# VealFang/PLI-SLAM

Measured on AMD Instinct MI355X. Metric: stereo frames/sec (ORB+LSD extract+match), 752x480 EuRoC, higher is better.
Workload: dtype u8; 1 GPU; 1xMI355X: 752x480 stereo pairs, extract + stereo Hamming match (BASELINE configs[1] shape, batched); 752x480, 1200 ORB kp (8 levels x1.2) + LSD/LBD (<=100 lines); 256 stereo frames per GPU per step; frames_per_gpu=256, parallelism=frame-batch data parallel, 1 rank(s), gather of result tables to rank 0

## Files before the change

### pli_slam_amd/csrc/kernels.hpp

```cpp
#pragma once
#include "common.hpp"

namespace pli {

struct BlurPlane {
  int w, h, pitchIn, pitchOut;
  int64_t offIn, offOut;
  int tilesX, tileBase;
};
struct BlurJob {
  int nplanes;
  BlurPlane pl[MAX_LEVELS];
  int k[7];
  int radius;
};
struct LbdCoef { float L[21]; float G[63]; };

constexpr signed char ORB_PATTERN_HOST[1024] = {
#include "../../include/pli_orb_pattern.inc"
};
constexpr int orbPatternReach() {
  int best = 0;
  for (int i = 0; i < 512; ++i) {
    const long long x = ORB_PATTERN_HOST[2 * i], y = ORB_PATTERN_HOST[2 * i + 1], r2 = x * x + y * y;
    int n = 0;
    while ((long long)(2 * n + 1) * (2 * n + 1) * 10000 <= 4 * r2 * 10002) ++n;
    best = n > best ? n : best;
  }
  return best;
}
constexpr int ORB_REACH = orbPatternReach();
constexpr int ORB_BLUR_R = 3;
constexpr int ORB_HALF_PATCH = 15;
constexpr int LBD_BLUR_R = 2;
constexpr int PROJ_K = 64;
__global__ void k_ingest_copy16(const uint8_t* __restrict__ left, const uint8_t* __restrict__ right, int64_t stride, int64_t frameStride, uint8_t* __restrict__ pyr, int64_t pyrBlock, int W16, int H, int pitch, int img0);
__global__ void k_ingest(const uint8_t* __restrict__ left, const uint8_t* __restrict__ right, int64_t stride, int64_t frameStride, uint8_t* __restrict__ pyr, int64_t pyrBlock, int W, int H, int pitch, const float2* __restrict__ mapL, const float2* __restrict__ mapR, int img0);
__global__ void k_resize_level(const uint8_t* __restrict__ srcBase, int64_t srcImgStride, int sw, int sh, int spitch, uint8_t* __restrict__ dstBase, int64_t dstImgStride, int dw, int dh, int dpitch, const int* __restrict__ tab, int img0);
__global__ void k_fast_cells(const DevParams* __restrict__ Pp, const uint8_t* __restrict__ pyr, uint32_t* __restrict__ cellCand, int* __restrict__ cellCount, int img0);
__global__ void k_octree(const DevParams* __restrict__ Pp, const uint32_t* __restrict__ cellCand, const int* __restrict__ cellCount, uint32_t* __restrict__ candAll, unsigned short* __restrict__ nodeOfAll, int* __restrict__ candCount, uint32_t* __restrict__ kpSel, int* __restrict__ kpSelCount, int img0);
__global__ void k_octree_512(const DevParams* __restrict__ Pp, const uint32_t* __restrict__ cellCand, const int* __restrict__ cellCount, uint32_t* __restrict__ candAll, unsigned short* __restrict__ nodeOfAll, int* __restrict__ candCount, uint32_t* __restrict__ kpSel, int* __restrict__ kpSelCount, int img0);
__global__ void k_octree_320(const DevParams* __restrict__ Pp, const uint32_t* __restrict__ cellCand, const int* __restrict__ cellCount, uint32_t* __restrict__ candAll, unsigned short* __restrict__ nodeOfAll, int* __restrict__ candCount, uint32_t* __restrict__ kpSel, int* __restrict__ kpSelCount, int img0);
__global__ void k_octree_w(const DevParams* __restrict__ Pp, const uint32_t* __restrict__ cellCand, const int* __restrict__ cellCount, uint32_t* __restrict__ candAll, unsigned short* __restrict__ nodeOfAll, int* __restrict__ candCount, uint32_t* __restrict__ kpSel, int* __restrict__ kpSelCount, int img0);
__global__ void k_octree_512_w(const DevParams* __restrict__ Pp, const uint32_t* __restrict__ cellCand, const int* __restrict__ cellCount, uint32_t* __restrict__ candAll, unsigned short* __restrict__ nodeOfAll, int* __restrict__ candCount, uint32_t* __restrict__ kpSel, int* __restrict__ kpSelCount, int img0);
__global__ void k_octree_320_w(const DevParams* __restrict__ Pp, const uint32_t* __restrict__ cellCand, const int* __restrict__ cellCount, uint32_t* __restrict__ candAll, unsigned short* __restrict__ nodeOfAll, int* __restrict__ candCount, uint32_t* __restrict__ kpSel, int* __restrict__ kpSelCount, int img0);
__global__ void k_blur(const BlurJob* __restrict__ Jp, const uint8_t* __restrict__ in, int64_t inImgStride, uint8_t* __restrict__ out, int64_t outImgStride, int img0);
__global__ void k_describe(const DevParams* __restrict__ Pp, const uint8_t* __restrict__ pyr, const BlurJob* __restrict__ Jp, const uint32_t* __restrict__ kpSel, const int* __restrict__ kpSelCount, uint8_t* __restrict__ table, int64_t recordBytes, int64_t offCounts, int64_t offKp0, int64_t offKp1, int64_t offDesc0, int64_t offDesc1, int img0);
__global__ void k_kp_counts(const DevParams* __restrict__ Pp, const int* __restrict__ kpSelCount, uint8_t* __restrict__ table, int64_t recordBytes, int64_t offCounts, int nimg, int img0);
__global__ void k_lsd_grad(const uint8_t* __restrict__ scaled, int64_t imgStride, int W, int H, int WP, int pitch, int g2Thresh, float4* __restrict__ rec, int* __restrict__ g2o, int2* __restrict__ own, int* __restrict__ maxG2, float* __restrict__ angDbg, int img0, int trigF32);
__global__ void k_lsd_hist(const int* __restrict__ g2a, int npix, int g2Thresh, int nBins, const int* __restrict__ maxG2, unsigned short* __restrict__ chunkHist, int nChunks, int img0, const double* __restrict__ mgAll, const unsigned long long* __restrict__ maxMg, double rho, const RxCtl* __restrict__ onlyUnsettled);
__global__ void k_lsd_scan(const unsigned short* __restrict__ chunkHist, int nChunks, int nBins, int* __restrict__ chunkBase, int* __restrict__ nDefined, int img0, const RxCtl* __restrict__ onlyUnsettled);
__global__ void k_lsd_scatter(const int* __restrict__ g2a, int npix, int g2Thresh, int nBins, const int* __restrict__ maxG2, const int* __restrict__ chunkBase, int nChunks, int* __restrict__ order, int img0, int nimg, const double* __restrict__ mgAll, const unsigned long long* __restrict__ maxMg, double rho, int* __restrict__ rankAll, const int* __restrict__ groupOff, int chunksPerGroup, int nGroups, const RxCtl* __restrict__ onlyUnsettled);
__global__ void k_lsd_scan_part(const unsigned short* __restrict__ chunkHist, int nChunks, int nBins, int chunksPerGroup, int* __restrict__ chunkBase, int* __restrict__ groupOff, int img0, const RxCtl* __restrict__ onlyUnsettled);
__global__ void k_lsd_scan_groups(int nGroups, int nBins, int* __restrict__ groupOff, int* __restrict__ nDefined, int img0, const RxCtl* __restrict__ onlyUnsettled);
__global__ void k_lsd_grow_unsettled(const DevParams* __restrict__ Pp, float4* __restrict__ recAll, const double* __restrict__ mgAll, const int* __restrict__ orderAll, const int* __restrict__ nDefined, uint2* __restrict__ regOverflow, float* __restrict__ segAll, int* __restrict__ nSeg, int maxSeg, int img0, int nimg, RxCtl* __restrict__ ctl);
__global__ void k_lsd_grow(const DevParams* __restrict__ Pp, float4* __restrict__ recAll, const double* __restrict__ mgAll, const int* __restrict__ orderAll, const int* __restrict__ nDefined, uint2* __restrict__ regOverflow, float* __restrict__ segAll, int* __restrict__ nSeg, int maxSeg, int img0, int nimg);
__global__ void k_lsd_grow2(const DevParams* __restrict__ Pp, float4* __restrict__ recAll, const double* __restrict__ mgAll, const int* __restrict__ orderAll, const int* __restrict__ nDefined, uint2* __restrict__ regOverflow, float* __restrict__ segAll, int* __restrict__ nSeg, int maxSeg, int img0, int nimg);
__global__ void k_lsd_grow_spec(const DevParams* __restrict__ Pp, float4* __restrict__ recAll, const double* __restrict__ mgAll, const int* __restrict__ orderAll, const int* __restrict__ nDefined, uint2* __restrict__ regOverflow, float* __restrict__ segAll, int* __restrict__ nSeg, int maxSeg, int img0, int nimg, LsdRectItem* __restrict__ rectAll, double* __restrict__ rectWAll);
__global__ void k_lsd_grow2_spec(const DevParams* __restrict__ Pp, float4* __restrict__ recAll, const double* __restrict__ mgAll, const int* __restrict__ orderAll, const int* __restrict__ nDefined, uint2* __restrict__ regOverflow, float* __restrict__ segAll, int* __restrict__ nSeg, int maxSeg, int img0, int nimg, LsdRectItem* __restrict__ rectAll, double* __restrict__ rectWAll);
__global__ void k_lsd_rect(const DevParams* __restrict__ Pp, const LsdRectItem* __restrict__ rectAll, const uint2* __restrict__ arenaAll, const double* __restrict__ mgAll, const double* __restrict__ rectWAll, const int* __restrict__ nSeg, float* __restrict__ segAll, int maxSeg, int img0);
__global__ void k_keylines(const DevParams* __restrict__ Pp, const float* __restrict__ seg, const int* __restrict__ nSeg, int maxSeg, pli_keyline* __restrict__ tmpKL, uint8_t* __restrict__ table, int64_t recordBytes, int64_t offCounts, int64_t offKl0, int64_t offKl1, int img0);
__global__ void k_sobel(const BlurJob* __restrict__ Jp, const uint8_t* __restrict__ in, int64_t inImgStride, short2* __restrict__ dxy, int img0);
__global__ void k_lbd(const DevParams* __restrict__ Pp, const LbdCoef* __restrict__ coef, const short2* __restrict__ dxya, uint8_t* __restrict__ table, int64_t recordBytes, int64_t offCounts, int64_t offKl0, int64_t offKl1, int64_t offLd0, int64_t offLd1, float* __restrict__ dbgFloat, int img0);
__global__ void k_lsd_blur64(const uint8_t* __restrict__ pyr, int64_t pyrBlock, int W, int H, int pitch, const double* __restrict__ kern, int radius, double* __restrict__ out, int64_t outImgStride, int img0);
__global__ void k_lsd_resize64(const double* __restrict__ src, int sw, int sh, double* __restrict__ dst, int dw, int dh, int64_t dstImgStride, const int* __restrict__ tab, int img0);
__global__ void k_lsd_grad64(const double* __restrict__ scaled, int W, int H, int WP, int64_t scaledImgStride, double rho, float4* __restrict__ rec, double* __restrict__ mg, int2* __restrict__ own, unsigned long long* __restrict__ maxMg, float* __restrict__ angDbg, int img0, int flags, int2* __restrict__ hot, float2* __restrict__ cold);
__global__ void k_lsd_front64(const uint8_t* __restrict__ pyr, int64_t pyrBlock, int sw, int sh, int pitch, const double* __restrict__ kern, int radius, const int* __restrict__ tab, int dw, int dh, int dp, double rho, float4* __restrict__ rec, double* __restrict__ mg, int2* __restrict__ own, unsigned long long* __restrict__ maxMg, int img0, int flags, int2* __restrict__ hot, float2* __restrict__ cold);
__global__ void k_rx_guess(const float4* __restrict__ recAll, const int* __restrict__ rankAll, int2* __restrict__ ownAll, int W, int H, float precDeg, int img0);
__global__ void k_rx_diff(RxCtl* __restrict__ ctl, const int2* __restrict__ ownAll, int* __restrict__ tileMinAll, int* __restrict__ tileActAll, int W, int H, int TW, int TH, int t, int img0, const int* __restrict__ tileTouchAll);
__global__ void k_rx_classify(RxCtl* __restrict__ ctl, const int2* __restrict__ ownAll, const int* __restrict__ rankAll, const int2* __restrict__ rgBoxAll, uint8_t* __restrict__ rgCleanAll, const int* __restrict__ tileMinAll, int W, int H, int TW, int TH, int t, int img0);
__global__ void k_rx_seed(RxCtl* __restrict__ ctl, int2* __restrict__ ownAll, const int* __restrict__ rankAll, const float4* __restrict__ recAll, const int* __restrict__ rgSizeAll, const uint8_t* __restrict__ rgCleanAll, RxSeed* __restrict__ smallAll, RxSeed* __restrict__ bigAll, int bigCap, int W, int H, int bigThresh, int t, int img0);
__global__ void k_rx_mark(RxCtl* __restrict__ ctl, const int2* __restrict__ ownAll, const int* __restrict__ rankAll, const int2* __restrict__ rgBoxAll, int* __restrict__ rgDirtyAll, const int* __restrict__ tileMinAll, int* __restrict__ tileActAll, int W, int H, int TW, int TH, int t, int img0, int seedRule, const int* __restrict__ rgLostAll, TxDirtyLists DL);
__global__ void k_rx_seed_sparse(RxCtl* __restrict__ ctl, int2* __restrict__ ownAll, const int* __restrict__ rankAll, const float4* __restrict__ recAll, const int* __restrict__ rgSizeAll, const int* __restrict__ rgDirtyAll, const int* __restrict__ tileActAll, RxSeed* __restrict__ smallAll, RxSeed* __restrict__ bigAll, int bigCap, int W, int H, int TW, int TH, int bigThresh, int t, int img0);
__global__ void k_rx_grow(const DevParams* __restrict__ Pp, RxCtl* __restrict__ ctl, const float4* __restrict__ recAll, int2* __restrict__ ownAll, const RxSeed* __restrict__ smallAll, int* __restrict__ rgSizeAll, int2* __restrict__ rgBoxAll, RxHand* __restrict__ handAll, int handCap, int* __restrict__ arenaAll, int arenaCap, RxRect* __restrict__ rectAll, int rectCap, int img0, int t);
__global__ void k_rx_grow_big(const DevParams* __restrict__ Pp, RxCtl* __restrict__ ctl, const float4* __restrict__ recAll, int2* __restrict__ ownAll, const RxSeed* __restrict__ bigAll, int bigCap, const RxHand* __restrict__ handAll, int handCap, int* __restrict__ rgSizeAll, int2* __restrict__ rgBoxAll, int* __restrict__ arenaAll, int arenaCap, RxRect* __restrict__ rectAll, int rectCap, int img0, int t);
__global__ void k_rx_grow_wave(const DevParams* __restrict__ Pp, RxCtl* __restrict__ ctl, const float4* __restrict__ recAll, int2* __restrict__ ownAll, const RxSeed* __restrict__ bigAll, int bigCap, const RxHand* __restrict__ handAll, int handCap, int* __restrict__ rgSizeAll, int2* __restrict__ rgBoxAll, int* __restrict__ arenaAll, int arenaCap, RxRect* __restrict__ rectAll, int rectCap, int img0, int t);
__global__ void k_rx_rect(const DevParams* __restrict__ Pp, RxCtl* __restrict__ ctl, const float4* __restrict__ recAll, const int* __restrict__ arenaAll, int arenaCap, const RxRect* __restrict__ rectAll, int rectCap, float4* __restrict__ rgSegAll, int img0, const double* __restrict__ mgAll, int rmask, const int2* __restrict__ hotAll, const float2* __restrict__ coldAll);
__global__ void k_rx_count(const RxCtl* __restrict__ ctl, const int* __restrict__ orderAll, const int* __restrict__ nDefined, const int2* __restrict__ ownAll, const int* __restrict__ rgSizeAll, int* __restrict__ chunkCntAll, int nChunks, int64_t npix, int minReg, int img0);
__global__ void k_rx_emit(const RxCtl* __restrict__ ctl, const int* __restrict__ orderAll, const int* __restrict__ nDefined, const int2* __restrict__ ownAll, const int* __restrict__ rgSizeAll, const float4* __restrict__ rgSegAll, const int* __restrict__ chunkCntAll, int nChunks, int64_t npix, int minReg, float* __restrict__ segAll, int* __restrict__ nSeg, int maxSeg, int img0);
__global__ void k_tx_sort(const int* __restrict__ rankAll, const int* __restrict__ orderAll, int2* __restrict__ ownAll, int2* __restrict__ listAll, int* __restrict__ tileCntAll, int W, int H, int ts, int ntx, int nty, int img0, TxKeys keys);
__global__ void k_tx_sort128(const int* __restrict__ rankAll, const int* __restrict__ orderAll, int2* __restrict__ ownAll, int2* __restrict__ listAll, int* __restrict__ tileCntAll, int W, int H, int ts, int ntx, int nty, int img0, TxKeys keys);
__global__ void k_tx_mark(RxCtl* __restrict__ ctl, const int2* __restrict__ ownAll, const int* __restrict__ rankAll, const int2* __restrict__ rgBoxAll, int* __restrict__ rgDirtyAll, const int* __restrict__ tileMinAll, int* __restrict__ tileActAll, int W, int H, int TW, int TH, int t, int img0, const int* __restrict__ rgLostAll, TxDirtyLists DL);
__global__ void k_tx_round2(RxCtl* __restrict__ ctl, int2* __restrict__ ownAll, const int* __restrict__ rankAll, const int* __restrict__ orderAll, const int2* __restrict__ rgBoxAll, int* __restrict__ rgDirtyAll, int* __restrict__ tileActAll, int W, int H, int TW, int TH, int t, int img0, const int* __restrict__ rgLostAll, TxDirtyLists DL, int* __restrict__ tileTouchAll, const float4* __restrict__ recPack, int keepRect, const int2* __restrict__ hotPack);
__global__ void k_tx_reset_rect(RxCtl* __restrict__ ctl, int nimg, int img0);
__global__ void k_tx_diffmark(RxCtl* __restrict__ ctl, const int2* __restrict__ ownAll, const int* __restrict__ rankAll, const int2* __restrict__ rgBoxAll, int* __restrict__ rgDirtyAll, int* __restrict__ tileActAll, const int* __restrict__ tileTouchAll, int W, int H, int TW, int TH, int t, int img0, const int* __restrict__ rgLostAll, TxDirtyLists DL);
__global__ void k_tx_diff2(RxCtl* __restrict__ ctl, const int2* __restrict__ ownAll, const int* __restrict__ orderAll, const int2* __restrict__ rgBoxAll, int* __restrict__ rgDirtyAll, int* __restrict__ tileMinAll, int* __restrict__ tileActAll, int W, int H, int TW, int TH, int ts, int t, int img0, const int* __restrict__ rgLostAll, TxDirtyLists DL);
__global__ void k_tx_prep(RxCtl* __restrict__ ctl, int2* __restrict__ ownAll, const int* __restrict__ rankAll, const int* __restrict__ rgDirtyAll, const int* __restrict__ tileActAll, int W, int H, int TW, int TH, int t, int img0, int full, int* __restrict__ tileTouchAll, int rmask, int stamp);
__global__ void k_tx_grow(const DevParams* __restrict__ Pp, RxCtl* __restrict__ ctl, const float4* __restrict__ recAll, int2* __restrict__ ownAll, const int2* __restrict__ listAll, const int* __restrict__ tileCntAll, int ts, int ntx, int nty, int* __restrict__ rgSizeAll, int2* __restrict__ rgBoxAll, const int* __restrict__ rgDirtyAll, const int* __restrict__ tileActAll, int TW, int TH, int* __restrict__ arenaAll, int arenaCap, RxRect* __restrict__ rectAll, int rectCap, int img0, int t, const int* __restrict__ rankAll, int* __restrict__ rgLostAll, int* __restrict__ tileTouchAll, TxDirtyLists DL);
__global__ void k_tx_grow_p1(const DevParams* __restrict__ Pp, RxCtl* __restrict__ ctl, float4* recAll, int2* __restrict__ ownAll, const int2* __restrict__ listAll, const int* __restrict__ tileCntAll, int ts, int ntx, int nty, int* __restrict__ rgSizeAll, int2* __restrict__ rgBoxAll, const int* __restrict__ rgDirtyAll, const int* __restrict__ tileActAll, int TW, int TH, int* __restrict__ arenaAll, int arenaCap, RxRect* __restrict__ rectAll, int rectCap, int img0, int t, const int* __restrict__ rankAll, int* __restrict__ rgLostAll, int* __restrict__ tileTouchAll, TxDirtyLists DL, TxKeys keys);
__global__ void k_tx_grow_p2(const DevParams* __restrict__ Pp, RxCtl* __restrict__ ctl, float4* recAll, int2* __restrict__ ownAll, const int2* __restrict__ listAll, const int* __restrict__ tileCntAll, int ts, int ntx, int nty, int* __restrict__ rgSizeAll, int2* __restrict__ rgBoxAll, const int* __restrict__ rgDirtyAll, const int* __restrict__ tileActAll, int TW, int TH, int* __restrict__ arenaAll, int arenaCap, RxRect* __restrict__ rectAll, int rectCap, int img0, int t, const int* __restrict__ rankAll, int* __restrict__ rgLostAll, int* __restrict__ tileTouchAll, TxDirtyLists DL, TxKeys keys);
__global__ void k_tx_grow_h1(const DevParams* __restrict__ Pp, RxCtl* __restrict__ ctl, const float4* __restrict__ recAll, int2* __restrict__ ownAll, const int2* __restrict__ listAll, const int* __restrict__ tileCntAll, int ts, int ntx, int nty, int* __restrict__ rgSizeAll, int2* __restrict__ rgBoxAll, const int* __restrict__ rgDirtyAll, const int* __restrict__ tileActAll, int TW, int TH, int* __restrict__ arenaAll, int arenaCap, RxRect* __restrict__ rectAll, int rectCap, int img0, int t, const int* __restrict__ rankAll, int* __restrict__ rgLostAll, int* __restrict__ tileTouchAll, TxDirtyLists DL, TxKeys keys);
__global__ void k_tx_grow_h2(const DevParams* __restrict__ Pp, RxCtl* __restrict__ ctl, const float4* __restrict__ recAll, int2* __restrict__ ownAll, const int2* __restrict__ listAll, const int* __restrict__ tileCntAll, int ts, int ntx, int nty, int* __restrict__ rgSizeAll, int2* __restrict__ rgBoxAll, const int* __restrict__ rgDirtyAll, const int* __restrict__ tileActAll, int TW, int TH, int* __restrict__ arenaAll, int arenaCap, RxRect* __restrict__ rectAll, int rectCap, int img0, int t, const int* __restrict__ rankAll, int* __restrict__ rgLostAll, int* __restrict__ tileTouchAll, TxDirtyLists DL, TxKeys keys);
__global__ void k_tx_grow_spec(const DevParams* __restrict__ Pp, RxCtl* __restrict__ ctl, const float4* __restrict__ recAll, int2* __restrict__ ownAll, const int2* __restrict__ listAll, const int* __restrict__ tileCntAll, int ts, int ntx, int nty, int* __restrict__ rgSizeAll, int2* __restrict__ rgBoxAll, const int* __restrict__ rgDirtyAll, const int* __restrict__ tileActAll, int TW, int TH, int* __restrict__ arenaAll, int arenaCap, RxRect* __restrict__ rectAll, int rectCap, int img0, int t, const int* __restrict__ rankAll, int* __restrict__ rgLostAll, int* __restrict__ tileTouchAll, TxDirtyLists DL);
__global__ void k_tx_grow_sparse(const DevParams* __restrict__ Pp, RxCtl* __restrict__ ctl, const float4* __restrict__ recAll, int2* __restrict__ ownAll, const int2* __restrict__ listAll, const int* __restrict__ tileCntAll, int ts, int ntx, int nty, int* __restrict__ rgSizeAll, int2* __restrict__ rgBoxAll, const int* __restrict__ rgDirtyAll, const int* __restrict__ tileActAll, int TW, int TH, int* __restrict__ arenaAll, int arenaCap, RxRect* __restrict__ rectAll, int rectCap, int img0, int t, const int* __restrict__ rankAll, int* __restrict__ rgLostAll, int* __restrict__ tileTouchAll, TxDirtyLists DL);
__global__ void k_tx_grow_sparse_h(const DevParams* __restrict__ Pp, RxCtl* __restrict__ ctl, const float4* __restrict__ recAll, int2* __restrict__ ownAll, const int2* __restrict__ listAll, const int* __restrict__ tileCntAll, int ts, int ntx, int nty, int* __restrict__ rgSizeAll, int2* __restrict__ rgBoxAll, const int* __restrict__ rgDirtyAll, const int* __restrict__ tileActAll, int TW, int TH, int* __restrict__ arenaAll, int arenaCap, RxRect* __restrict__ rectAll, int rectCap, int img0, int t, const int* __restrict__ rankAll, int* __restrict__ rgLostAll, int* __restrict__ tileTouchAll, TxDirtyLists DL, int2* __restrict__ hotAll, const float2* __restrict__ coldAll);
__global__ void k_stereo_points(const DevParams* __restrict__ Pp, const uint8_t* __restrict__ pyr, uint8_t* __restrict__ table, int64_t recordBytes, int64_t offCounts, int64_t offKp0, int64_t offKp1, int64_t offDesc0, int64_t offDesc1, int64_t offUr, int64_t offDepth, int* __restrict__ sadOut, int* __restrict__ bestIdxOut);
__global__ void k_stereo_median(const DevParams* __restrict__ Pp, uint8_t* __restrict__ table, int64_t recordBytes, int64_t offCounts, int64_t offUr, int64_t offDepth, const int* __restrict__ sadIn);
__global__ void k_stereo_lines(const DevParams* __restrict__ Pp, uint8_t* __restrict__ table, int64_t recordBytes, int64_t offCounts, int64_t offKl0, int64_t offKl1, int64_t offLd0, int64_t offLd1, int64_t offDisp, int64_t offLe, unsigned long long* __restrict__ maskAll, double* __restrict__ dirAll, short* __restrict__ dmatAll, int* __restrict__ m12All, int* __restrict__ m21All, int phase);
__global__ void k_distance(const uint8_t* __restrict__ a, const uint8_t* __restrict__ b, int n, int* __restrict__ out);
__global__ void k_knn2(const uint8_t* __restrict__ q, int nq, const uint8_t* __restrict__ t, int nt, int* __restrict__ idx, int* __restrict__ dist);
__global__ void k_ratio(const int* __restrict__ idx, const int* __restrict__ dist, int n, int nTrain, float nnr, int* __restrict__ m);
__global__ void k_mutual(int* __restrict__ m12, const int* __restrict__ m21, int n1, int* __restrict__ nmatches);
__global__ void k_stereo_from_depth(const DevParams* __restrict__ Pp, const float* __restrict__ depthImg, int64_t pitch, int W, int H, uint8_t* __restrict__ table, int64_t offCounts, int64_t offKp0, int64_t offUr, int64_t offDepth);
__global__ void k_proj_candidates(const pli_proj_query* __restrict__ q, const uint8_t* __restrict__ qdesc, int nq, const pli_keypoint* __restrict__ kp, const uint8_t* __restrict__ desc, const float* __restrict__ uright, int ncur, float minX, float maxX, float minY, float maxY, int checkBounds, int distLimit, unsigned long long* __restrict__ candKeys, int* __restrict__ candCount);
__global__ void k_proj_assign(const pli_proj_query* __restrict__ q, const uint8_t* __restrict__ qdesc, int nq, const pli_keypoint* __restrict__ kp, const uint8_t* __restrict__ desc, const float* __restrict__ uright, const uint8_t* __restrict__ occupied, int ncur, float minX, float maxX, float minY, float maxY, int mode, int checkOri, float nnratio, const unsigned long long* __restrict__ candKeys, const int* __restrict__ candCount, int* __restrict__ bestIdx2, int* __restrict__ nmatchesOut, int* __restrict__ rawIdx2);
__global__ void k_proj_assign_scan(const pli_proj_query* __restrict__ q, const uint8_t* __restrict__ qdesc, int nq, const pli_keypoint* __restrict__ kp, const uint8_t* __restrict__ desc, const float* __restrict__ uright, const uint8_t* __restrict__ occupied, int ncur, float minX, float maxX, float minY, float maxY, int mode, int checkOri, float nnratio, int* __restrict__ owner , int* __restrict__ bestIdx2, int* __restrict__ nmatchesOut, int* __restrict__ rawIdx2);
__global__ void k_track_queries(const DevParams* __restrict__ Pp, const uint8_t* __restrict__ table, const float* __restrict__ poses, TrackParams tp, pli_proj_query* __restrict__ qAll);
__global__ void k_track_candidates(const uint8_t* __restrict__ table, TrackParams tp, const pli_proj_query* __restrict__ qAll, unsigned long long* __restrict__ candKeysAll, int* __restrict__ candCountAll);
__global__ void k_track_assign(const uint8_t* __restrict__ table, TrackParams tp, const pli_proj_query* __restrict__ qAll, const unsigned long long* __restrict__ candKeysAll, const int* __restrict__ candCountAll, uint8_t* __restrict__ track);
__global__ void k_track_lines(const uint8_t* __restrict__ table, TrackParams tp, int bestLR, int* __restrict__ scratch, uint8_t* __restrict__ track);
__global__ void k_bow_descend(const uint8_t* __restrict__ feat, int n, const int* __restrict__ childOff, const int* __restrict__ childList, const uint8_t* __restrict__ nodeDesc, const int* __restrict__ nodeWord, const double* __restrict__ nodeWeight, int nidLevel, int* __restrict__ wordId, double* __restrict__ weight, int* __restrict__ nodeId);
__global__ void k_node_sort(const int* __restrict__ kfOff, int nkOne, const int* __restrict__ kfNode, const uint8_t* __restrict__ kfFlag, int flagWanted, const uint8_t* __restrict__ kfStereo, int onlyStereo, int keyCap, uint32_t* __restrict__ sNode, uint16_t* __restrict__ sIdx, int* __restrict__ nListed, int* __restrict__ stat);
__global__ void k_search_by_bow(const int* __restrict__ kfOff, const uint8_t* __restrict__ kfDesc, const float* __restrict__ kfAngle, const int* __restrict__ kfNode, const uint8_t* __restrict__ kfValid, const uint8_t* __restrict__ fDesc, const float* __restrict__ fAngle, const uint32_t* __restrict__ sNode, const uint16_t* __restrict__ sIdx, const int* __restrict__ nListed, int nf, int keyCap, float nnratio, int checkOri, int* __restrict__ matches, int* __restrict__ nmatchesOut);
__global__ void k_tri_match(const pli_keypoint* __restrict__ kp1, const uint8_t* __restrict__ desc1, const int* __restrict__ node1, const uint8_t* __restrict__ hasMp1, const uint8_t* __restrict__ stereo1, int n1, const int* __restrict__ kfOff, const pli_keypoint* __restrict__ kfKp, const uint8_t* __restrict__ kfDesc, const uint8_t* __restrict__ kfStereo, const uint32_t* __restrict__ sNode, const uint16_t* __restrict__ sIdx, const int* __restrict__ nListed, const float* __restrict__ F12, const float* __restrict__ ep, const float* __restrict__ scaleFactor, const float* __restrict__ sigma2, int onlyStereo, int coarse, int checkOri, int* __restrict__ matches12, int* __restrict__ stat);
__global__ void k_tri_finish(const pli_keypoint* __restrict__ kp1, int n1, const int* __restrict__ kfOff, const pli_keypoint* __restrict__ kfKp, int* __restrict__ matches12, int* __restrict__ stat);
__global__ void k_search_by_bow_kf(const uint8_t* __restrict__ desc1, const float* __restrict__ angle1, const int* __restrict__ node1, const uint8_t* __restrict__ valid1, int n1, const int* __restrict__ kfOff, const uint8_t* __restrict__ kfDesc, const float* __restrict__ kfAngle, const uint32_t* __restrict__ sNode, const uint16_t* __restrict__ sIdx, const int* __restrict__ nListed, int keyCap, float nnratio, int checkOri, int* __restrict__ matches12, int* __restrict__ nmatchesOut);
struct FuseSurvivor { int kf, mp; float u, v, ur, radius; int level, pad; };
__global__ void k_fuse_grid(const int* __restrict__ kfOff, const pli_keypoint* __restrict__ kfKp, pli_fuse_camera cam, int* __restrict__ cellStart, uint16_t* __restrict__ sIdx);
// ... 22 lines not shown
```

### pli_slam_amd/csrc/match_kernels.hip

```cpp
#include "kernels.hpp"
#include "device_prims.hpp"
#include <climits>

namespace pli {

__device__ __forceinline__ void load_desc(const uint8_t* p, uint64_t d[4]) {
  const uint64_t* q = reinterpret_cast<const uint64_t*>(p);
  d[0] = q[0]; d[1] = q[1]; d[2] = q[2]; d[3] = q[3];
}

constexpr int HISTO_LENGTH = 30;

__device__ __forceinline__ int rot_bin(float a, float b) {
  float rot = __fsub_rn(a, b);
  if (rot < 0.0f) rot = __fadd_rn(rot, 360.0f);
  int bin = (int)roundf(__fmul_rn(rot, 1.0f / HISTO_LENGTH));
  if (bin == HISTO_LENGTH) bin = 0;
  return bin;
}

__device__ __forceinline__ void three_maxima(const int* hist, int& ind1, int& ind2, int& ind3) {
  int max1 = 0, max2 = 0, max3 = 0, i1 = -1, i2 = -1, i3 = -1;
  for (int i = 0; i < HISTO_LENGTH; i++) {
    const int s = hist[i];
    if (s > max1) { max3 = max2; max2 = max1; max1 = s; i3 = i2; i2 = i1; i1 = i; }
    else if (s > max2) { max3 = max2; max2 = s; i3 = i2; i2 = i; }
    else if (s > max3) { max3 = s; i3 = i; }
  }
  if ((float)max2 < __fmul_rn(0.1f, (float)max1)) { i2 = -1; i3 = -1; }
  else if ((float)max3 < __fmul_rn(0.1f, (float)max1)) i3 = -1;
  ind1 = i1; ind2 = i2; ind3 = i3;
}

__global__ __launch_bounds__(64) void k_stereo_points(const DevParams* __restrict__ Pp, const uint8_t* __restrict__ pyr,
                                                      uint8_t* __restrict__ table, int64_t recordBytes,
                                                      int64_t offCounts, int64_t offKp0, int64_t offKp1,
                                                      int64_t offDesc0, int64_t offDesc1, int64_t offUr,
                                                      int64_t offDepth, int* __restrict__ sadOut,
                                                      int* __restrict__ bestIdxOut) {
  const DevParams& P = *Pp;
  const int frame = blockIdx.y, iL = blockIdx.x, lane = threadIdx.x;
  uint8_t* rec = table + (int64_t)frame * recordBytes;
  const int* counts = reinterpret_cast<const int*>(rec + offCounts);
  const int N = counts[0], Nr = counts[1];
  if (iL >= N) return;
  const pli_keypoint* kpsL = reinterpret_cast<const pli_keypoint*>(rec + offKp0);
  const pli_keypoint* kpsR = reinterpret_cast<const pli_keypoint*>(rec + offKp1);
  const uint8_t* descL = rec + offDesc0;
  const uint8_t* descR = rec + offDesc1;
  float* uright = reinterpret_cast<float*>(rec + offUr);
  float* depth = reinterpret_cast<float*>(rec + offDepth);
  const pli_keypoint kpL = kpsL[iL];
  const int levelL = kpL.octave;
  const float vL = kpL.y, uL = kpL.x;
  const int rowL = (int)vL;
  const float maxD = P.maxD, minD = 0.f;
  const float minU = __fsub_rn(uL, maxD), maxU = __fsub_rn(uL, minD);
  uint64_t dL[4];
  load_desc(descL + (int64_t)iL * 32, dL);
  unsigned long long bestKey = ~0ull;
  __shared__ float s_r[MAX_LEVELS];
  if (lane < MAX_LEVELS) s_r[lane] = lane < P.nlevels ? __fmul_rn(2.0f, P.lv[lane].scale) : 0.f;
  __syncthreads();
  if (!(maxU < 0)) {
#pragma unroll 4
    for (int iR = lane; iR < Nr; iR += 64) {
      const pli_keypoint kpR = kpsR[iR];
      const float r = s_r[kpR.octave];
      const int maxr = (int)ceilf(__fadd_rn(kpR.y, r));
      const int minr = (int)floorf(__fsub_rn(kpR.y, r));
      if (rowL < minr || rowL > maxr) continue;
      if (kpR.octave < levelL - 1 || kpR.octave > levelL + 1) continue;
      const float uR = kpR.x;
      if (uR >= minU && uR <= maxU) {
        uint64_t dR[4];
        load_desc(descR + (int64_t)iR * 32, dR);
        const int dist = hamming256(dL, dR);
        if (dist < 100) {
          unsigned long long key = ((unsigned long long)dist << 32) | (unsigned)iR;
          bestKey = key < bestKey ? key : bestKey;
        }
      }
    }
  }
  bestKey = wave_min_u64(bestKey);
  float outU = -1.f, outD = -1.f;
  int outSad = -1, outIdx = -1;
  const int thOrbDist = (100 + 50) / 2;
  if (bestKey != ~0ull && (int)(bestKey >> 32) < thOrbDist) {
    const int bestIdxR = (int)(bestKey & 0xFFFFFFFFu);
    outIdx = bestIdxR;
    const float uR0 = kpsR[bestIdxR].x;
    const LevelGeom& G = P.lv[levelL];
    const float scaleFactor = G.invScale;
    const float scaleduL = roundf(__fmul_rn(kpL.x, scaleFactor));
    const float scaledvL = roundf(__fmul_rn(kpL.y, scaleFactor));
    const float scaleduR0 = roundf(__fmul_rn(uR0, scaleFactor));
    const int w = 5, L = 5;
    const int cy = (int)scaledvL, cxl = (int)scaleduL, cxr = (int)scaleduR0;
    bool ok = !(cy - w < 0 || cy + w + 1 > G.h || cxl - w < 0 || cxl + w + 1 > G.w);
    const float iniu = __fadd_rn(scaleduR0, (float)(L - w));
    const float endu = __fadd_rn(scaleduR0, (float)(L + w + 1));
    if (iniu < 0 || endu >= (float)G.w) ok = false;
    if (cxr - L - w < 0) ok = false;
    if (ok) {
      const uint8_t* imL = pyr + (int64_t)(frame * 2) * P.pyrBlock + G.offset;
      const uint8_t* imR = pyr + (int64_t)(frame * 2 + 1) * P.pyrBlock + G.offset;
      const int cL = imL[(int64_t)cy * G.pitch + cxl];
      int aL[2], px[2], py[2];
      bool act[2];
#pragma unroll
      for (int k = 0; k < 2; ++k) {
        int i = lane + 64 * k;
        act[k] = i < 121;
        int dy = act[k] ? i / 11 - w : 0, dx = act[k] ? i % 11 - w : 0;
        px[k] = dx; py[k] = dy;
        aL[k] = act[k] ? (int)imL[(int64_t)(cy + dy) * G.pitch + cxl + dx] - cL : 0;
      }
      float vDists[11];
      int bestDist = INT_MAX, bestincR = 0;
#pragma unroll
      for (int incR = -L; incR <= L; ++incR) {
        const int cR = imR[(int64_t)cy * G.pitch + cxr + incR];
        int s = 0;
#pragma unroll
        for (int k = 0; k < 2; ++k)
          if (act[k]) {
            int b = (int)imR[(int64_t)(cy + py[k]) * G.pitch + cxr + incR + px[k]] - cR;
            s += abs(aL[k] - b);
          }
        s = wave_sum_i32(s);
        const float dist = (float)s;
        if (dist < (float)bestDist) { bestDist = (int)dist; bestincR = incR; }
        vDists[L + incR] = dist;
      }
      if (!(bestincR == -L || bestincR == L)) {
        float dist1 = 0, dist2 = 0, dist3 = 0;
#pragma unroll
        for (int k = 1; k < 10; ++k)
          if (k == L + bestincR) { dist1 = vDists[k - 1]; dist2 = vDists[k]; dist3 = vDists[k + 1]; }
        const float deltaR = __fdiv_rn(__fsub_rn(dist1, dist3),
                                       __fmul_rn(2.0f, __fsub_rn(__fadd_rn(dist1, dist3), __fmul_rn(2.0f, dist2))));
        if (!(deltaR < -1 || deltaR > 1)) {
          float bestuR = __fmul_rn(G.scale, __fadd_rn(__fadd_rn(scaleduR0, (float)bestincR), deltaR));
          float disparity = __fsub_rn(uL, bestuR);
          if (disparity >= minD && disparity < maxD) {
            if (disparity <= 0) {
              disparity = 0.01f;
              bestuR = (float)((double)uL - 0.01);
            }
            outD = __fdiv_rn(P.bf, disparity);
            outU = bestuR;
            outSad = bestDist;
          }
        }
      }
    }
  }
  if (lane == 0) {
    uright[iL] = outU;
    depth[iL] = outD;
    sadOut[(int64_t)frame * P.kpCap + iL] = outSad;
    if (bestIdxOut) bestIdxOut[(int64_t)frame * P.kpCap + iL] = outIdx;
  }
}

__global__ __launch_bounds__(256) void k_stereo_median(const DevParams* __restrict__ Pp, uint8_t* __restrict__ table,
                                                       int64_t recordBytes, int64_t offCounts, int64_t offUr,
                                                       int64_t offDepth, const int* __restrict__ sadIn) {
  extern __shared__ int s_sad[];
  __shared__ int s_m, s_median, s_left;
  const DevParams& P = *Pp;
  const int frame = blockIdx.x, tid = threadIdx.x;
  uint8_t* rec = table + (int64_t)frame * recordBytes;
  int* counts = reinterpret_cast<int*>(rec + offCounts);
  const int N = counts[0];
  float* uright = reinterpret_cast<float*>(rec + offUr);
  float* depth = reinterpret_cast<float*>(rec + offDepth);
  const int* sad = sadIn + (int64_t)frame * P.kpCap;
  if (tid == 0) { s_m = 0; s_median = -1; s_left = 0; }
  __syncthreads();
  int loc = 0;
  for (int i = tid; i < N; i += 256) {
    int v = sad[i];
    s_sad[i] = v;
    loc += v >= 0;
  }
  if (loc) atomicAdd(&s_m, loc);
  __syncthreads();
  const int M = s_m;
  if (M == 0) {
    if (tid == 0) counts[4] = 0;
    return;
  }
  __shared__ int s_hist[256];
  __shared__ unsigned s_pref, s_mask;
  __shared__ int s_k;
  if (tid == 0) { s_pref = 0u; s_mask = 0u; s_k = M / 2; }
  for (int shift = 24; shift >= 0; shift -= 8) {
    s_hist[tid] = 0;
    __syncthreads();
    const unsigned pref = s_pref, mask = s_mask;
    for (int i = tid; i < N; i += 256) {
      const int v = s_sad[i];
      if (v >= 0 && ((unsigned)v & mask) == pref) atomicAdd(&s_hist[((unsigned)v >> shift) & 255u], 1);
    }
    __syncthreads();
    if (tid < 64) {
      const int h0 = s_hist[4 * tid], h1 = s_hist[4 * tid + 1], h2 = s_hist[4 * tid + 2], h3 = s_hist[4 * tid + 3];
      const int sum = h0 + h1 + h2 + h3;
      int inc = sum;
#pragma unroll
      for (int o = 1; o < 64; o <<= 1) {
        const int t2 = __shfl_up(inc, o, 64);
        if (tid >= o) inc += t2;
      }
      const int k = s_k, before = inc - sum;
      if (before <= k && k < inc) {
        int b = 0, c = before;
        if (k >= c + h0) { c += h0; b = 1; if (k >= c + h1) { c += h1; b = 2; if (k >= c + h2) { c += h2; b = 3; } } }
        s_pref = pref | ((unsigned)(4 * tid + b) << shift);
        s_mask = mask | (255u << shift);
        s_k = k - c;
      }
    }
    __syncthreads();
  }
  if (tid == 0) s_median = (int)s_pref;
  __syncthreads();
  const float median = (float)s_median;
  const float thDist = __fmul_rn(__fmul_rn(1.5f, 1.4f), median);
  loc = 0;
  for (int i = tid; i < N; i += 256) {
    const int v = s_sad[i];
    if (v < 0) continue;
    if (!((float)v < thDist)) {
      uright[i] = -1.f;
      depth[i] = -1.f;
    } else ++loc;
  }
  if (loc) atomicAdd(&s_left, loc);
  __syncthreads();
  if (tid == 0) counts[4] = s_left;
}

__device__ __forceinline__ void normalize2(double& a, double& b) {
// ... 1552 lines not shown
```

### pli_slam_amd/csrc/pli_capi.hip

```cpp
#include "kernels.hpp"
#include "scratch_plan.hpp"
#include <cmath>
#include <cfloat>
#include <algorithm>
#include <memory>
#include <limits>
#include <cstdlib>
#include <set>
#include <string>
#include <functional>
#include <mutex>
#include <atomic>
#include <dlfcn.h>

using namespace pli;

#ifdef PLI_DEV
#define DEVENV(name) getenv(name)
#else
static inline const char* pli_no_devenv() { return nullptr; }
#define DEVENV(name) (pli_no_devenv())
#endif

namespace {
// ... 1233 lines not shown
      if (nimg <= 4)
        TRL(c, "k_rx_grow_wave", k_rx_grow_wave, dim3(bigBlocks * 4, nimg), dim3(64), 0, c->dP, c->jrCtl, c->rec, c->own, c->bigSeeds,
            c->bigCap, c->hand, c->handCap, c->lastSize, c->rgBox, c->arena, c->arenaCap, c->rects, c->rectCap, img0, t);
      else
        TRL(c, "k_rx_grow_big", k_rx_grow_big, dim3(bigBlocks, nimg), dim3(64), 0, c->dP, c->jrCtl, c->rec, c->own, c->bigSeeds,
            c->bigCap, c->hand, c->handCap, c->lastSize, c->rgBox, c->arena, c->arenaCap, c->rects, c->rectCap, img0, t);
      TRL(c, "k_rx_rect", k_rx_rect, dim3(rectBlocks, nimg), dim3(64), 0, c->dP, c->jrCtl, c->rec, c->arena, c->arenaCap, c->rects,
          c->rectCap, c->rgSeg, img0, c->mg, -1, (const int2*)nullptr, (const float2*)nullptr);
      if (trace) {
        HIPCHK(hipMemcpyAsync(c->jrHost.data(), c->jrCtl + img0, sizeof(RxCtl) * nimg, hipMemcpyDeviceToHost, c->stream));
        HIPCHK(hipStreamSynchronize(c->stream));
        const RxCtl& h = c->jrHost[0];
        std::fprintf(stderr, "[rx] t=%d state=%d changed=%d overflow=%d small=%d big=%d hand=%d nextBig=%d rect=%d arena=%lld races=%d\n", t,
                     h.state, h.changed, h.overflow, h.nSmall, h.nBig, h.nHand, h.nextBig, (int)(h.rectArena >> RX_ARENA_BITS),
                     (long long)(h.rectArena & ((1ull << RX_ARENA_BITS) - 1ull)), h.races);
      }
      { pli_status ls_ = look(t); if (ls_ != PLI_OK) return ls_; }
    }
#endif
    }
    if (keyMode) {
      int emitCap = TX_EMIT_CAP;
      if (const char* e = DEVENV("PLI_TX_EMITCAP")) emitCap = std::max(1, std::min(TX_EMIT_CAP, atoi(e)));
      TRL(c, "k_tx_collect", k_tx_collect, dim3(std::max(1, std::min(64, (int)((npix64 + 2047) / 2048))), nimg), dim3(256), 0, c->jrCtl,
          (const int*)c->rankOf, (const int2*)c->own, (const int*)c->lastSize, npix64, P.minRegSize, c->txCand, c->txCandCnt, img0, emitCap);
      TRL(c, "k_tx_emit_sorted", k_tx_emit_sorted, dim3(nimg), dim3(1024), TX_EMIT_CAP * 4, (const RxCtl*)c->jrCtl, (const int*)c->txCand,
          (const int*)c->txCandCnt, (const float4*)c->rgSeg, npix64, (1 << c->txPixBits) - 1, c->seg, c->nSeg, c->maxSeg, img0, emitCap);
      pli_status os = orderPasses(c->jrCtl);
      if (os != PLI_OK) return os;
    } else {
    TRL(c, "k_rx_count", k_rx_count, dim3(c->rxChunks, nimg), dim3(256), 0, c->jrCtl, c->order, c->nDefined, c->own, c->lastSize,
           c->rxChunkCnt, c->rxChunks, npix64, P.minRegSize, img0);
    TRL(c, "k_rx_emit", k_rx_emit, dim3(c->rxChunks, nimg), dim3(256), 0, c->jrCtl, c->order, c->nDefined, c->own, c->lastSize,
           c->rgSeg, c->rxChunkCnt, c->rxChunks, npix64, P.minRegSize, c->seg, c->nSeg, c->maxSeg, img0);
    }
    if (hotAll)
      LAUNCH(c, "k_tx_rec_from_hot", k_tx_rec_from_hot, dim3(std::max(1, std::min(64, (int)((npix64 + 4095) / 4096))), nimg), dim3(256), 0,
             (const RxCtl*)c->jrCtl, (const int2*)c->hot, (const float2*)c->cold, c->rec, npix64, img0);
    if (blocking && !keyMode) {
      for (int i = 0; i < nimg; ++i) {
        if (c->jrHost[i].overflow || c->jrHost[i].state != 2) {
          LAUNCH(c, "k_lsd_grow", k_lsd_grow, dim3(1), dim3(64), 0, c->dP, c->rec, c->mg, c->order, c->nDefined,
                 c->regScratch, c->seg, c->nSeg, c->maxSeg, img0 + i, 1);
        }
      }
    } else {
      LAUNCH(c, "k_lsd_grow_unsettled", k_lsd_grow_unsettled, dim3(nimg), dim3(64), 0, c->dP, c->rec, c->mg, c->order, c->nDefined,
             c->regScratch, c->seg, c->nSeg, c->maxSeg, img0, nimg, c->jrCtl);
      if (!blocking) {
      if (!c->rxSeen) {
        HIPCHK(hipHostMalloc((void**)&c->rxSeen, sizeof(int) * (4 * (size_t)c->NI + 1), hipHostMallocDefault));
        c->rxSeen[4 * (size_t)c->NI] = 0;
        HIPCHK(hipEventCreateWithFlags(&c->evRxSeen, hipEventDisableTiming));
      }
      if (c->rxSeenImages == 0) {
        HIPCHK(hipMemcpy2DAsync(c->rxSeen, 16, c->jrCtl + img0, sizeof(RxCtl), 16, nimg, hipMemcpyDeviceToHost, c->stream));
        if (c->tailBar && c->tailLaunched)
          HIPCHK(hipMemcpyAsync(c->rxSeen + 4 * (size_t)c->NI, c->tailBar + 32, sizeof(int), hipMemcpyDeviceToHost, c->stream));
        else c->rxSeen[4 * (size_t)c->NI] = 0;
        HIPCHK(hipEventRecord(c->evRxSeen, c->stream));
        c->rxSeenImages = nimg;
        c->rxSeenTail = c->tailLaunched;
      }
      }
    }
  }
  LAUNCH(c, "k_keylines", k_keylines, dim3(nimg), dim3(256), 0, c->dP, c->seg, c->nSeg, c->maxSeg, c->tmpKL, table,
         Y.record_bytes, Y.off_counts, Y.off_kl[0], Y.off_kl[1], img0);
  if (c->lbdPreOnSide) {
    HIPCHK(hipStreamWaitEvent(c->stream, c->evLbdPre, 0));
  } else {
    pli_status ls = runLbdPre(c, img0, nimg);
    if (ls != PLI_OK) return ls;
  }
  LAUNCH(c, "k_lbd", k_lbd, dim3(P.klCap, nimg), dim3(64), 0, c->dP, c->lbdCoef, c->dxy, table, Y.record_bytes,
         Y.off_counts, Y.off_kl[0], Y.off_kl[1], Y.off_ldesc[0], Y.off_ldesc[1], c->debug ? c->lbdFloat : (float*)nullptr, img0);
  return PLI_OK;
}

pli_status runStereoPoints(pli_ctx* c, int nframes, uint8_t* table) {
  TraceRange range__("pli:stereo points");
  const DevParams& P = c->hp;
  const pli_table_layout& Y = c->lay;
  LAUNCH(c, "k_stereo_points", k_stereo_points, dim3(P.kpCap, nframes), dim3(64), 0, c->dP, c->pyr, table, Y.record_bytes,
         Y.off_counts, Y.off_kp[0], Y.off_kp[1], Y.off_desc[0], Y.off_desc[1], Y.off_uright, Y.off_depth, c->sad,
         c->debug ? c->bestIdx : (int*)nullptr);
  LAUNCH(c, "k_stereo_median", k_stereo_median, dim3(nframes), dim3(256), (size_t)P.kpCap * 4, c->dP, table, Y.record_bytes,
         Y.off_counts, Y.off_uright, Y.off_depth, c->sad);
  return PLI_OK;
}

pli_status runStereoLines(pli_ctx* c, int nframes, uint8_t* table) {
  TraceRange range__("pli:stereo lines");
  const pli_table_layout& Y = c->lay;
  const int cap = c->hp.klCap;
  const int slices = (cap >= 192 && !DEVENV("PLI_STEREO_LINES_1")) ? std::max(1, std::min(64, (cap * cap) / 8192)) : 1;
  for (int phase = slices > 1 ? 1 : 0; phase <= (slices > 1 ? 3 : 0); ++phase)
    LAUNCH(c, "k_stereo_lines", k_stereo_lines, dim3(nframes, phase == 2 ? slices : 1), dim3(256), 0, c->dP, table, Y.record_bytes,
           Y.off_counts, Y.off_kl[0], Y.off_kl[1], Y.off_ldesc[0], Y.off_ldesc[1], Y.off_disp, Y.off_le, c->lmask, c->ldir, c->dmat,
           c->m12, c->m21, phase);
  return PLI_OK;
}

pli_status ensureScratch(pli_ctx* c, size_t bytes) {
  if (bytes <= c->scratchBytes) return PLI_OK;
  if (c->scratch) hipFree(c->scratch);
  c->scratch = nullptr; c->scratchBytes = 0;
  HIPCHK(hipMalloc(&c->scratch, bytes));
  c->scratchBytes = bytes;
  return PLI_OK;
}

pli_status commitScratch(pli_ctx* c, ScratchPlan& plan) {
  const pli_status st = ensureScratch(c, plan.bytes());
  if (st == PLI_OK) plan.bind(c->scratch);
  return st;
}

template <typename T>
hipError_t upload(pli_ctx* c, ScratchBlock<T> dst, const T* src, size_t n) {
  return n ? hipMemcpyAsync(dst, src, n * sizeof(T), hipMemcpyHostToDevice, c->stream) : hipSuccess;
}
template <typename T>
hipError_t download(pli_ctx* c, T* dst, ScratchBlock<T> src, size_t n) {
  return dst && n ? hipMemcpyAsync(dst, src, n * sizeof(T), hipMemcpyDeviceToHost, c->stream) : hipSuccess;
}

pli_status fetchCount(pli_ctx* c, const int* dcount, int32_t* nmatches) {
  int cnt = 0;
  HIPCHK(hipMemcpyAsync(&cnt, dcount, 4, hipMemcpyDeviceToHost, c->stream));
  HIPCHK(hipStreamSynchronize(c->stream));
  if (nmatches) *nmatches = cnt;
  return PLI_OK;
}

struct RecordCounts {
  int32_t kp[2], kl[2];
  int32_t stereoPoints, stereoLines;
  uint8_t linesCut[2], kpCut[2];
  int32_t reserved;
};
static_assert(sizeof(RecordCounts) == 32 && offsetof(RecordCounts, linesCut) == 24, "the int32[8] at off_counts");

pli_status readCounts(pli_ctx* c, RecordCounts& rc) {
  HIPCHK(hipMemcpyAsync(&rc, c->ownTable + c->lay.off_counts, sizeof(rc), hipMemcpyDeviceToHost, c->stream));
  HIPCHK(hipStreamSynchronize(c->stream));
  return PLI_OK;
}

template <typename T>
hipError_t copyColumn(pli_ctx* c, T* dst, int64_t off, int n, int per = 1) {
  return dst && n > 0 ? hipMemcpy(dst, c->ownTable + off, (size_t)n * per * sizeof(T), hipMemcpyDeviceToHost) : hipSuccess;
}

pli_status checkImage(pli_ctx* c, const uint8_t* img, int w, int h, int64_t stride) {
  if (!img || w <= 0 || h <= 0) { g_err = "empty image"; return PLI_ERR_EMPTY_IMAGE; }
  if (w != c->cfg.width || h != c->cfg.height) { g_err = "image size differs from the context's"; return PLI_ERR_INVALID; }
  if (stride < w) { g_err = "stride < width"; return PLI_ERR_INVALID; }
  return PLI_OK;
}

pli_status stageImage(pli_ctx* c, int eye, const uint8_t* img, int w, int h, int64_t stride) {
  HIPCHK(hipMemcpy2DAsync(c->inStage[eye], w, img, stride, w, h, hipMemcpyHostToDevice, c->stream));
  return runIngest(c, c->inStage[0], c->inStage[1], w, 0, eye, 1);
}

struct KfBatch {
// ... 1633 lines not shown
```

Baseline: 6457 stereo frames/s.

## Tile stereo point matching: share right-keypoint attributes in LDS across 32 left keypoints

After: 6463 stereo frames/s, median of 5. About the same (+0.1%).

```diff
diff --git a/pli_slam_amd/csrc/kernels.hpp b/pli_slam_amd/csrc/kernels.hpp
--- a/pli_slam_amd/csrc/kernels.hpp
+++ b/pli_slam_amd/csrc/kernels.hpp
@@ -34,6 +34,9 @@
 constexpr int ORB_HALF_PATCH = 15;
 constexpr int LBD_BLUR_R = 2;
 constexpr int PROJ_K = 64;
+constexpr int SP_BLOCK = 32;
+constexpr int SP_THREADS = 256;
+constexpr int SP_CHUNK = 1280;
 __global__ void k_ingest_copy16(const uint8_t* __restrict__ left, const uint8_t* __restrict__ right, int64_t stride, int64_t frameStride, uint8_t* __restrict__ pyr, int64_t pyrBlock, int W16, int H, int pitch, int img0);
 __global__ void k_ingest(const uint8_t* __restrict__ left, const uint8_t* __restrict__ right, int64_t stride, int64_t frameStride, uint8_t* __restrict__ pyr, int64_t pyrBlock, int W, int H, int pitch, const float2* __restrict__ mapL, const float2* __restrict__ mapR, int img0);
 __global__ void k_resize_level(const uint8_t* __restrict__ srcBase, int64_t srcImgStride, int sw, int sh, int spitch, uint8_t* __restrict__ dstBase, int64_t dstImgStride, int dw, int dh, int dpitch, const int* __restrict__ tab, int img0);
diff --git a/pli_slam_amd/csrc/match_kernels.hip b/pli_slam_amd/csrc/match_kernels.hip
--- a/pli_slam_amd/csrc/match_kernels.hip
+++ b/pli_slam_amd/csrc/match_kernels.hip
@@ -32,136 +32,162 @@
   ind1 = i1; ind2 = i2; ind3 = i3;
 }
 
-__global__ __launch_bounds__(64) void k_stereo_points(const DevParams* __restrict__ Pp, const uint8_t* __restrict__ pyr,
-                                                      uint8_t* __restrict__ table, int64_t recordBytes,
-                                                      int64_t offCounts, int64_t offKp0, int64_t offKp1,
-                                                      int64_t offDesc0, int64_t offDesc1, int64_t offUr,
-                                                      int64_t offDepth, int* __restrict__ sadOut,
-                                                      int* __restrict__ bestIdxOut) {
+__global__ __launch_bounds__(SP_THREADS) void k_stereo_points(const DevParams* __restrict__ Pp, const uint8_t* __restrict__ pyr,
+                                                              uint8_t* __restrict__ table, int64_t recordBytes,
+                                                              int64_t offCounts, int64_t offKp0, int64_t offKp1,
+                                                              int64_t offDesc0, int64_t offDesc1, int64_t offUr,
+                                                              int64_t offDepth, int* __restrict__ sadOut,
+                                                              int* __restrict__ bestIdxOut) {
+  __shared__ int s_minr[SP_CHUNK], s_maxr[SP_CHUNK], s_oct[SP_CHUNK];
+  __shared__ float s_x[SP_CHUNK];
+  __shared__ float s_r[MAX_LEVELS];
+  __shared__ unsigned long long s_best[SP_BLOCK];
   const DevParams& P = *Pp;
-  const int frame = blockIdx.y, iL = blockIdx.x, lane = threadIdx.x;
+  const int frame = blockIdx.y, iL0 = blockIdx.x * SP_BLOCK, tid = threadIdx.x, lane = tid & 63;
+  const int wv = __builtin_amdgcn_readfirstlane(tid >> 6);
   uint8_t* rec = table + (int64_t)frame * recordBytes;
   const int* counts = reinterpret_cast<const int*>(rec + offCounts);
   const int N = counts[0], Nr = counts[1];
-  if (iL >= N) return;
+  if (iL0 >= N) return;
+  const int nL = min(SP_BLOCK, N - iL0);
   const pli_keypoint* kpsL = reinterpret_cast<const pli_keypoint*>(rec + offKp0);
   const pli_keypoint* kpsR = reinterpret_cast<const pli_keypoint*>(rec + offKp1);
   const uint8_t* descL = rec + offDesc0;
   const uint8_t* descR = rec + offDesc1;
   float* uright = reinterpret_cast<float*>(rec + offUr);
   float* depth = reinterpret_cast<float*>(rec + offDepth);
-  const pli_keypoint kpL = kpsL[iL];
-  const int levelL = kpL.octave;
-  const float vL = kpL.y, uL = kpL.x;
-  const int rowL = (int)vL;
   const float maxD = P.maxD, minD = 0.f;
-  const float minU = __fsub_rn(uL, maxD), maxU = __fsub_rn(uL, minD);
-  uint64_t dL[4];
-  load_desc(descL + (int64_t)iL * 32, dL);
-  unsigned long long bestKey = ~0ull;
-  __shared__ float s_r[MAX_LEVELS];
-  if (lane < MAX_LEVELS) s_r[lane] = lane < P.nlevels ? __fmul_rn(2.0f, P.lv[lane].scale) : 0.f;
-  __syncthreads();
-  if (!(maxU < 0)) {
+  if (tid < MAX_LEVELS) s_r[tid] = tid < P.nlevels ? __fmul_rn(2.0f, P.lv[tid].scale) : 0.f;
+  if (tid < SP_BLOCK) s_best[tid] = ~0ull;
+  for (int base = 0; base < Nr; base += SP_CHUNK) {
+    __syncthreads();
+    const int m = min(SP_CHUNK, Nr - base);
+    for (int i = tid; i < m; i += SP_THREADS) {
+      const pli_keypoint kpR = kpsR[base + i];
+      const float r = s_r[kpR.octave];
+      s_maxr[i] = (int)ceilf(__fadd_rn(kpR.y, r));
+      s_minr[i] = (int)floorf(__fsub_rn(kpR.y, r));
+      s_oct[i] = kpR.octave;
+      s_x[i] = kpR.x;
+    }
+    __syncthreads();
+    for (int j = wv; j < nL; j += SP_THREADS / 64) {
+      const int iL = iL0 + j;
+      const pli_keypoint kpL = kpsL[iL];
+      const int levelL = kpL.octave;
+      const int rowL = (int)kpL.y;
+      const float minU = __fsub_rn(kpL.x, maxD), maxU = __fsub_rn(kpL.x, minD);
+      if (maxU < 0) continue;
+      uint64_t dL[4];
+      load_desc(descL + (int64_t)iL * 32, dL);
+      unsigned long long bestKey = ~0ull;
 #pragma unroll 4
-    for (int iR = lane; iR < Nr; iR += 64) {
-      const pli_keypoint kpR = kpsR[iR];
-      const float r = s_r[kpR.octave];
-      const int maxr = (int)ceilf(__fadd_rn(kpR.y, r));
-      const int minr = (int)floorf(__fsub_rn(kpR.y, r));
-      if (rowL < minr || rowL > maxr) continue;
-      if (kpR.octave < levelL - 1 || kpR.octave > levelL + 1) continue;
-      const float uR = kpR.x;
-      if (uR >= minU && uR <= maxU) {
-        uint64_t dR[4];
-        load_desc(descR + (int64_t)iR * 32, dR);
-        const int dist = hamming256(dL, dR);
-        if (dist < 100) {
-          unsigned long long key = ((unsigned long long)dist << 32) | (unsigned)iR;
-          bestKey = key < bestKey ? key : bestKey;
-        }
-      }
-    }
-  }
-  bestKey = wave_min_u64(bestKey);
-  float outU = -1.f, outD = -1.f;
-  int outSad = -1, outIdx = -1;
-  const int thOrbDist = (100 + 50) / 2;
-  if (bestKey != ~0ull && (int)(bestKey >> 32) < thOrbDist) {
-    const int bestIdxR = (int)(bestKey & 0xFFFFFFFFu);
-    outIdx = bestIdxR;
-    const float uR0 = kpsR[bestIdxR].x;
-    const LevelGeom& G = P.lv[levelL];
-    const float scaleFactor = G.invScale;
-    const float scaleduL = roundf(__fmul_rn(kpL.x, scaleFactor));
-    const float scaledvL = roundf(__fmul_rn(kpL.y, scaleFactor));
-    const float scaleduR0 = roundf(__fmul_rn(uR0, scaleFactor));
-    const int w = 5, L = 5;
-    const int cy = (int)scaledvL, cxl = (int)scaleduL, cxr = (int)scaleduR0;
-    bool ok = !(cy - w < 0 || cy + w + 1 > G.h || cxl - w < 0 || cxl + w + 1 > G.w);
-    const float iniu = __fadd_rn(scaleduR0, (float)(L - w));
-    const float endu = __fadd_rn(scaleduR0, (float)(L + w + 1));
-    if (iniu < 0 || endu >= (float)G.w) ok = false;
-    if (cxr - L - w < 0) ok = false;
-    if (ok) {
-      const uint8_t* imL = pyr + (int64_t)(frame * 2) * P.pyrBlock + G.offset;
-      const uint8_t* imR = pyr + (int64_t)(frame * 2 + 1) * P.pyrBlock + G.offset;
-      const int cL = imL[(int64_t)cy * G.pitch + cxl];
-      int aL[2], px[2], py[2];
-      bool act[2];
-#pragma unroll
-      for (int k = 0; k < 2; ++k) {
-        int i = lane + 64 * k;
-        act[k] = i < 121;
-        int dy = act[k] ? i / 11 - w : 0, dx = act[k] ? i % 11 - w : 0;
-        px[k] = dx; py[k] = dy;
-        aL[k] = act[k] ? (int)imL[(int64_t)(cy + dy) * G.pitch + cxl + dx] - cL : 0;
-      }
-      float vDists[11];
-      int bestDist = INT_MAX, bestincR = 0;
-#pragma unroll
-      for (int incR = -L; incR <= L; ++incR) {
-        const int cR = imR[(int64_t)cy * G.pitch + cxr + incR];
-        int s = 0;
-#pragma unroll
-        for (int k = 0; k < 2; ++k)
-          if (act[k]) {
-            int b = (int)imR[(int64_t)(cy + py[k]) * G.pitch + cxr + incR + px[k]] - cR;
-            s += abs(aL[k] - b);
-          }
-        s = wave_sum_i32(s);
-        const float dist = (float)s;
-        if (dist < (float)bestDist) { bestDist = (int)dist; bestincR = incR; }
-        vDists[L + incR] = dist;
-      }
-      if (!(bestincR == -L || bestincR == L)) {
-        float dist1 = 0, dist2 = 0, dist3 = 0;
-#pragma unroll
-        for (int k = 1; k < 10; ++k)
-          if (k == L + bestincR) { dist1 = vDists[k - 1]; dist2 = vDists[k]; dist3 = vDists[k + 1]; }
-        const float deltaR = __fdiv_rn(__fsub_rn(dist1, dist3),
-                                       __fmul_rn(2.0f, __fsub_rn(__fadd_rn(dist1, dist3), __fmul_rn(2.0f, dist2))));
-        if (!(deltaR < -1 || deltaR > 1)) {
-          float bestuR = __fmul_rn(G.scale, __fadd_rn(__fadd_rn(scaleduR0, (float)bestincR), deltaR));
-          float disparity = __fsub_rn(uL, bestuR);
-          if (disparity >= minD && disparity < maxD) {
-            if (disparity <= 0) {
-              disparity = 0.01f;
-              bestuR = (float)((double)uL - 0.01);
-            }
-            outD = __fdiv_rn(P.bf, disparity);
-            outU = bestuR;
-            outSad = bestDist;
+      for (int i = lane; i < m; i += 64) {
+        if (rowL < s_minr[i] || rowL > s_maxr[i]) continue;
+        const int octR = s_oct[i];
+        if (octR < levelL - 1 || octR > levelL + 1) continue;
+        const float uR = s_x[i];
+        if (uR >= minU && uR <= maxU) {
+          const int iR = base + i;
+          uint64_t dR[4];
+          load_desc(descR + (int64_t)iR * 32, dR);
+          const int dist = hamming256(dL, dR);
+          if (dist < 100) {
+            unsigned long long key = ((unsigned long long)dist << 32) | (unsigned)iR;
+            bestKey = key < bestKey ? key : bestKey;
           }
         }
       }
-    }
-  }
-  if (lane == 0) {
-    uright[iL] = outU;
-    depth[iL] = outD;
-    sadOut[(int64_t)frame * P.kpCap + iL] = outSad;
-    if (bestIdxOut) bestIdxOut[(int64_t)frame * P.kpCap + iL] = outIdx;
+      bestKey = wave_min_u64(bestKey);
+      if (lane == 0 && bestKey < s_best[j]) s_best[j] = bestKey;
+    }
+  }
+  __syncthreads();
+  for (int j = wv; j < nL; j += SP_THREADS / 64) {
+    const int iL = iL0 + j;
+    const unsigned long long bestKey = s_best[j];
+    const pli_keypoint kpL = kpsL[iL];
+    const int levelL = kpL.octave;
+    const float uL = kpL.x;
+    float outU = -1.f, outD = -1.f;
+    int outSad = -1, outIdx = -1;
+    const int thOrbDist = (100 + 50) / 2;
+    if (bestKey != ~0ull && (int)(bestKey >> 32) < thOrbDist) {
+      const int bestIdxR = (int)(bestKey & 0xFFFFFFFFu);
+      outIdx = bestIdxR;
+      const float uR0 = kpsR[bestIdxR].x;
+      const LevelGeom& G = P.lv[levelL];
+      const float scaleFactor = G.invScale;
+      const float scaleduL = roundf(__fmul_rn(kpL.x, scaleFactor));
+      const float scaledvL = roundf(__fmul_rn(kpL.y, scaleFactor));
+      const float scaleduR0 = roundf(__fmul_rn(uR0, scaleFactor));
+      const int w = 5, L = 5;
+      const int cy = (int)scaledvL, cxl = (int)scaleduL, cxr = (int)scaleduR0;
+      bool ok = !(cy - w < 0 || cy + w + 1 > G.h || cxl - w < 0 || cxl + w + 1 > G.w);
+      const float iniu = __fadd_rn(scaleduR0, (float)(L - w));
+      const float endu = __fadd_rn(scaleduR0, (float)(L + w + 1));
+      if (iniu < 0 || endu >= (float)G.w) ok = false;
+      if (cxr - L - w < 0) ok = false;
+      if (ok) {
+        const uint8_t* imL = pyr + (int64_t)(frame * 2) * P.pyrBlock + G.offset;
+        const uint8_t* imR = pyr + (int64_t)(frame * 2 + 1) * P.pyrBlock + G.offset;
+        const int cL = imL[(int64_t)cy * G.pitch + cxl];
+        int aL[2], px[2], py[2];
+        bool act[2];
+#pragma unroll
+        for (int k = 0; k < 2; ++k) {
+          int i = lane + 64 * k;
+          act[k] = i < 121;
+          int dy = act[k] ? i / 11 - w : 0, dx = act[k] ? i % 11 - w : 0;
+          px[k] = dx; py[k] = dy;
+          aL[k] = act[k] ? (int)imL[(int64_t)(cy + dy) * G.pitch + cxl + dx] - cL : 0;
+        }
+        float vDists[11];
+        int bestDist = INT_MAX, bestincR = 0;
+#pragma unroll
+        for (int incR = -L; incR <= L; ++incR) {
+          const int cR = imR[(int64_t)cy * G.pitch + cxr + incR];
+          int s = 0;
+#pragma unroll
+          for (int k = 0; k < 2; ++k)
+            if (act[k]) {
+              int b = (int)imR[(int64_t)(cy + py[k]) * G.pitch + cxr + incR + px[k]] - cR;
+              s += abs(aL[k] - b);
+            }
+          s = wave_sum_i32(s);
+          const float dist = (float)s;
+          if (dist < (float)bestDist) { bestDist = (int)dist; bestincR = incR; }
+          vDists[L + incR] = dist;
+        }
+        if (!(bestincR == -L || bestincR == L)) {
+          float dist1 = 0, dist2 = 0, dist3 = 0;
+#pragma unroll
+          for (int k = 1; k < 10; ++k)
+            if (k == L + bestincR) { dist1 = vDists[k - 1]; dist2 = vDists[k]; dist3 = vDists[k + 1]; }
+          const float deltaR = __fdiv_rn(__fsub_rn(dist1, dist3),
+                                         __fmul_rn(2.0f, __fsub_rn(__fadd_rn(dist1, dist3), __fmul_rn(2.0f, dist2))));
+          if (!(deltaR < -1 || deltaR > 1)) {
+            float bestuR = __fmul_rn(G.scale, __fadd_rn(__fadd_rn(scaleduR0, (float)bestincR), deltaR));
+            float disparity = __fsub_rn(uL, bestuR);
+            if (disparity >= minD && disparity < maxD) {
+              if (disparity <= 0) {
+                disparity = 0.01f;
+                bestuR = (float)((double)uL - 0.01);
+              }
+              outD = __fdiv_rn(P.bf, disparity);
+              outU = bestuR;
+              outSad = bestDist;
+            }
+          }
+        }
+      }
+    }
+    if (lane == 0) {
+      uright[iL] = outU;
+      depth[iL] = outD;
+      sadOut[(int64_t)frame * P.kpCap + iL] = outSad;
+      if (bestIdxOut) bestIdxOut[(int64_t)frame * P.kpCap + iL] = outIdx;
+    }
   }
 }
 
diff --git a/pli_slam_amd/csrc/pli_capi.hip b/pli_slam_amd/csrc/pli_capi.hip
--- a/pli_slam_amd/csrc/pli_capi.hip
+++ b/pli_slam_amd/csrc/pli_capi.hip
@@ -1339,7 +1339,7 @@
   TraceRange range__("pli:stereo points");
   const DevParams& P = c->hp;
   const pli_table_layout& Y = c->lay;
-  LAUNCH(c, "k_stereo_points", k_stereo_points, dim3(P.kpCap, nframes), dim3(64), 0, c->dP, c->pyr, table, Y.record_bytes,
+  LAUNCH(c, "k_stereo_points", k_stereo_points, dim3((P.kpCap + SP_BLOCK - 1) / SP_BLOCK, nframes), dim3(SP_THREADS), 0, c->dP, c->pyr, table, Y.record_bytes,
          Y.off_counts, Y.off_kp[0], Y.off_kp[1], Y.off_desc[0], Y.off_desc[1], Y.off_uright, Y.off_depth, c->sad,
          c->debug ? c->bestIdx : (int*)nullptr);
   LAUNCH(c, "k_stereo_median", k_stereo_median, dim3(nframes), dim3(256), (size_t)P.kpCap * 4, c->dP, table, Y.record_bytes,
```
